# Orange-OpenSource/AIVC

Hardware: AMD Instinct MI355X
Metric: encode+decode fps @1080p YUV420 (RA GOP32) (higher is better)
Workload: dtype f32; 1 GPU; 1920x1080 8-bit YUV420, coding structure 1_GOP_32: one 128-frame clip = 4 intra-period units of 33 frames (132 coded frames, the last 4 repeat the last frame) encoded + decoded per step; synthetic random-init stand-in for model ms_ssim-4 (widths {'n2': 64, 'n': 128, 'c_y': 64, 'c_short': 64, 'c_z': 32, 'n_h': 128}), last analysis conv calibrated so that 6 (MOFNet) / 12 (CodecNet) of the 64 y featu; parallelism=single GPU

## Files before the change

### aivc_amd/csrc/conv_wino.hip

```cpp
#include <stdlib.h>

#include "mfma_util.h"

namespace aivc {

struct WinoArgs {
  aivc_conv_params p;
  int TH, TW;
  int nby, nbx;
  int gy;
  int total;
  int poly;
  int cpp_shift;
};

constexpr int WINO_RAW_STAGE = 11 * 1024;
constexpr int WINO_U_STAGE = 32 * 1024;
constexpr int WINO_V_QUAD = 1152;
constexpr int WINO_V_POS = 2 * WINO_V_QUAD;
constexpr int WINO_V_STAGE = 16 * WINO_V_POS;
constexpr int WINO_LDS = 2 * (WINO_RAW_STAGE + WINO_U_STAGE + WINO_V_STAGE);

__device__ __attribute__((aligned(4096))) float wino_zeros[1024];

template <int MODE>
__host__ __device__ constexpr bool wino_zero_pos(int pc, int i, int j) {
  if constexpr (MODE == 1) return ((pc >> 1) && i == 3) || ((pc & 1) && j == 3);
  if constexpr (MODE == 2) return ((pc >> 1) && i == 0) || ((pc & 1) && j == 0);
  return false;
}
template <int MODE>
__host__ __device__ constexpr uint32_t wino_pos_mask(int pc, int half) {
  uint32_t m = 0u;
  for (int q = 0; q < 8; ++q) m |= wino_zero_pos<MODE>(pc, 2 * half + (q >> 2), q & 3) ? 0u : 1u << q;
  return m;
}

struct WinoWalk {
  uint32_t x_lo, x_hi, slot, wg_per_xcd;
  __device__ __forceinline__ WinoWalk(uint32_t total, uint32_t nwg, uint32_t wg) {
    const uint32_t xcd = wg & 7u;
    slot = wg >> 3;
    const uint32_t per_xcd = (total + 7u) >> 3;
    wg_per_xcd = (nwg + 7u - xcd) >> 3;
    x_lo = xcd * per_xcd;
    x_hi = min(x_lo + per_xcd, total);
  }
  __device__ __forceinline__ uint32_t block_of(uint32_t k) const { return x_lo + slot + k * wg_per_xcd; }
  __device__ __forceinline__ uint32_t count() const { return x_lo + slot < x_hi ? (x_hi - x_lo - slot + wg_per_xcd - 1u) / wg_per_xcd : 0u; }
};

template <int MODE>
__global__ __launch_bounds__(512) void conv_wino_kernel(WinoArgs a) {
  constexpr bool POLY = MODE == 1, TC = MODE == 2;
  extern __shared__ __attribute__((aligned(16))) char wsmem[];
  char *raw = wsmem, *Us = wsmem + 2 * WINO_RAW_STAGE, *Vs = Us + 2 * WINO_U_STAGE;
  const uint32_t lds0 = (uint32_t)(uintptr_t)(__attribute__((address_space(3))) char *)wsmem;

  const aivc_conv_params &p = a.p;
  const int tid = threadIdx.x, lane = tid & 63;
  const int wave = __builtin_amdgcn_readfirstlane(tid >> 6);
  const int ph = wave >> 2, wm = (wave >> 1) & 1, wn = wave & 1;
  const int H = TC ? p.h_in : p.h_out, W = TC ? p.w_in : p.w_out, Hi = p.h_in, Wi = p.w_in, Cin = p.c_in, Cout = p.c_out;
  const int gyc = TC ? 4 * a.gy : a.gy;
  const int cpp_shift = a.cpp_shift, cpp_mask = (1 << a.cpp_shift) - 1;

  const WinoWalk walk((uint32_t)a.total, gridDim.x, blockIdx.x);
  const uint32_t n_mine = walk.count();
  if (n_mine == 0u) return;
  struct Desc {
    const float *xbase, *ubase;
    uint32_t r_off[2];
    int img, byi, bxi, cb;
  };
  int s_quad[2], s_py[2], s_px[2];
#pragma unroll
  for (int k = 0; k < 2; ++k) {
    int sl = 64 * (wave + 8 * k) + lane;
    sl = sl < 648 ? sl : 647;
    const int q2 = sl >> 1, plane = q2 / 81, rem = q2 - plane * 81, hy = rem / 9, hx = rem - hy * 9;
    s_quad[k] = sl & 1;
    s_py[k] = 2 * hy + (plane >> 1);
    s_px[k] = 2 * hx + (plane & 1);
  }
  const int nch = POLY ? 4 * (Cin >> 3) : (Cin >> 3);
  auto make_desc = [&](uint32_t blk) {
    Desc d;
    d.cb = (int)(blk % (uint32_t)gyc);
    uint32_t rest = blk / (uint32_t)gyc;
    d.bxi = (int)(rest % (uint32_t)a.nbx);
    rest /= (uint32_t)a.nbx;
    d.byi = (int)(rest % (uint32_t)a.nby);
    d.img = (int)(rest / (uint32_t)a.nby);
    d.xbase = p.x + (size_t)d.img * (size_t)Hi * Wi * Cin;
    d.ubase = p.w_wino + (size_t)d.cb * (size_t)nch * (WINO_U_STAGE / 4);
    if constexpr (MODE == 0) {
#pragma unroll
      for (int k = 0; k < 2; ++k) {
        const int iy = max(min(16 * d.byi - 1 + s_py[k], Hi - 1), 0), ix = max(min(16 * d.bxi - 1 + s_px[k], Wi - 1), 0);
        d.r_off[k] = ((uint32_t)(iy * Wi + ix) * (uint32_t)Cin + (uint32_t)(4 * s_quad[k])) * 4u;
      }
    }
    return d;
  };
  uint32_t iss_off[2];
  auto patch_offsets = [&](const Desc &d_, int ph2) {
    const int st = POLY ? 2 : 1, py = ph2 >> 1, px = ph2 & 1;
#pragma unroll
    for (int k = 0; k < 2; ++k) {
      const int iy = max(min(st * (16 * d_.byi - 1 + s_py[k]) + py, Hi - 1), 0), ix = max(min(st * (16 * d_.bxi - 1 + s_px[k]) + px, Wi - 1), 0);
      iss_off[k] = ((uint32_t)(iy * Wi + ix) * (uint32_t)Cin + (uint32_t)(4 * s_quad[k])) * 4u;
    }
  };
  uint64_t iss_addr[2];
  auto tc_addresses = [&](const Desc &d_) {
#pragma unroll
    for (int k = 0; k < 2; ++k) {
      const int iy = 16 * d_.byi - 1 + s_py[k], ix = 16 * d_.bxi - 1 + s_px[k];
      const bool in = iy >= 0 && iy < Hi && ix >= 0 && ix < Wi;
      const uint64_t a_in = (uint64_t)(uintptr_t)d_.xbase + ((uint64_t)((uint32_t)(iy * Wi + ix)) * (uint32_t)Cin + (uint32_t)(4 * s_quad[k])) * 4u;
      const uint64_t a_z = (uint64_t)(uintptr_t)wino_zeros + (uint32_t)(16 * s_quad[k]);
      iss_addr[k] = in ? a_in : a_z;
    }
  };
  Desc cur = make_desc(walk.block_of(0)), nxt = n_mine > 1u ? make_desc(walk.block_of(1)) : cur;

  const uint32_t r_dst = __builtin_amdgcn_readfirstlane(lds0 + (uint32_t)wave * 1024u);
  const uint32_t u_dst = __builtin_amdgcn_readfirstlane(lds0 + (uint32_t)(2 * WINO_RAW_STAGE) + (uint32_t)wave * 4096u);
  const uint32_t u_off = (uint32_t)(wave * 4096 + lane * 16);
  auto uniform_ptr = [](const float *q) -> const float * {
    const uint64_t v = (uint64_t)(uintptr_t)q;
    const uint32_t lo = __builtin_amdgcn_readfirstlane((uint32_t)v), hi = __builtin_amdgcn_readfirstlane((uint32_t)(v >> 32));
    return reinterpret_cast<const float *>((uintptr_t)(((uint64_t)hi << 32) | lo));
  };
  auto issue_raw = [&](const Desc &d_, int c) {
    const uint32_t d = r_dst + (uint32_t)((c & 1) * WINO_RAW_STAGE);
    if constexpr (TC) {
      if (c == 0) tc_addresses(d_);
      const uint32_t du = __builtin_amdgcn_readfirstlane(d);
      asm volatile("s_mov_b32 m0, %1\n\ts_nop 0\n\tglobal_load_lds_dwordx4 %0, off" : : "v"(iss_addr[0]), "s"(du) : "memory", "m0");
      if (wave < 3) asm volatile("s_mov_b32 m0, %1\n\ts_nop 0\n\tglobal_load_lds_dwordx4 %0, off" : : "v"(iss_addr[1]), "s"(du + 8192u) : "memory", "m0");
      iss_addr[0] += 32u;
      iss_addr[1] += 32u;
    } else {
      const float *src = d_.xbase + 8 * c;
      glds16(src, d_.r_off[0], d);
      if (wave < 3) glds16(src, d_.r_off[1], d + 8192u);
    }
  };
  auto issue_u = [&](const Desc &d_, int c) {
    const float *src = TC ? uniform_ptr(d_.ubase + (size_t)c * (WINO_U_STAGE / 4)) : d_.ubase + (size_t)c * (WINO_U_STAGE / 4);
    const uint32_t d = TC ? __builtin_amdgcn_readfirstlane(u_dst + (uint32_t)((c & 1) * WINO_U_STAGE)) : u_dst + (uint32_t)((c & 1) * WINO_U_STAGE);
    bool lo = true, hi = true;
    if constexpr (TC) {
      const int cls = d_.cb / a.gy, i = wave >> 1, j = 2 * (wave & 1);
      lo = !wino_zero_pos<MODE>(cls, i, j);
      hi = !wino_zero_pos<MODE>(cls, i, j + 1);
    }
    if (lo && hi) glds_piece<GLDS_BOTH>(src, u_off, d);
    else if (lo) glds_piece<GLDS_LO>(src, u_off, d);
    else if (hi) glds_piece<GLDS_HI>(src, u_off, d);
  };

  struct Prep {
    const float *r_src, *u_src;
    uint32_t flags;
  };
  auto prepare = [&](uint32_t kb, int cr, int cu) -> Prep {
    Prep q;
    const bool more = kb + 1u < n_mine;
    uint32_t fl = 0u;
    {
      const bool own = cr < nch;
      const int c = own ? cr : cr - nch;
      const Desc &d_ = own ? cur : nxt;
      if (own || more) {
        fl |= 1u;
        if ((c & cpp_mask) == 0) patch_offsets(d_, c >> cpp_shift);
      }
      q.r_src = uniform_ptr(d_.xbase + 8 * (c & cpp_mask));
    }
    {
      const bool own = cu < nch;
      const int c = own ? cu : cu - nch;
      const Desc &d_ = own ? cur : nxt;
      q.u_src = uniform_ptr(d_.ubase + (size_t)c * (WINO_U_STAGE / 4));
      if (own || more) {
        const int pc = c >> cpp_shift, i = wave >> 1, j = 2 * (wave & 1);
        if (!wino_zero_pos<MODE>(pc, i, j)) fl |= 2u;
        if (!wino_zero_pos<MODE>(pc, i, j + 1)) fl |= 4u;
      }
    }
    q.flags = __builtin_amdgcn_readfirstlane(fl);
    return q;
  };
  auto fire_raw = [&](auto STAGE, const Prep &q) {
    const uint32_t d = r_dst + (uint32_t)(decltype(STAGE)::value * WINO_RAW_STAGE);
    if (q.flags & 1u) {
      glds16(q.r_src, iss_off[0], d);
      if (wave < 3) glds16(q.r_src, iss_off[1], d + 8192u);
    }
  };
  auto fire_u = [&](auto STAGE, const Prep &q) {
    const uint32_t d = u_dst + (uint32_t)(decltype(STAGE)::value * WINO_U_STAGE);
    const uint32_t both = q.flags & 6u;
    if (both == 6u) glds_piece<GLDS_BOTH>(q.u_src, u_off, d);
    else if (both == 2u) glds_piece<GLDS_LO>(q.u_src, u_off, d);
    else if (both == 4u) glds_piece<GLDS_HI>(q.u_src, u_off, d);
  };

  const int l32 = lane & 31;
  const int t_grp = (l32 < 4 || (l32 >= 12 && l32 < 16) || (l32 >= 20 && l32 < 28)) ? 0 : 1;
  const int t_pos = t_grp == 0 ? (l32 < 4 ? l32 : (l32 < 16 ? l32 - 8 : l32 - 12)) : (l32 < 12 ? l32 - 4 : (l32 < 20 ? l32 - 8 : l32 - 16));
  const int t_quad = t_pos >> 3, t_tx = (t_pos & 7) ^ (t_grp << 2), t_ty = ((tid >> 6) & 1) * 4 + (lane >> 5) * 2 + t_grp;
  const int t_i = __builtin_amdgcn_readfirstlane(tid >> 7);
  const int t_ra = t_i == 0 ? 0 : (t_i == 2 ? 2 : 1), t_rb = t_i == 3 ? 3 : (t_i == 2 ? 1 : 2);
  const float t_si = t_i == 1 ? 1.0f : -1.0f;
  const int t_base = ((t_ty * 9 + t_tx) * 2 + t_quad) * 16;
  auto pix_off = [](int r, int c) { return (((r & 1) * 2 + (c & 1)) * 81 + (r >> 1) * 9 + (c >> 1)) * 32; };
  int t_oa[4], t_ob[4];
#pragma unroll
  for (int c = 0; c < 4; ++c) {
    t_oa[c] = t_base + pix_off(t_ra, c);
    t_ob[c] = t_base + pix_off(t_rb, c);
  }
  const int t_vdst = (4 * t_i) * WINO_V_POS + t_quad * WINO_V_QUAD + (t_ty * 8 + t_tx) * 16;
  float4 R[4];
  auto comb = [](const float4 &u, const float4 &v, float sgn) {
    float4 o;
    o.x = __builtin_fmaf(sgn, v.x, u.x);
    o.y = __builtin_fmaf(sgn, v.y, u.y);
    o.z = __builtin_fmaf(sgn, v.z, u.z);
    o.w = __builtin_fmaf(sgn, v.w, u.w);
    return o;
  };
  auto transform_step = [&](auto STAGE, auto STEP) {
    constexpr int st = decltype(STEP)::value, stage = decltype(STAGE)::value;
    const char *rs = raw + stage * WINO_RAW_STAGE;
    char *vd = Vs + stage * WINO_V_STAGE + t_vdst;
    if constexpr (st < 4) {
      const float4 xa = *reinterpret_cast<const float4 *>(rs + t_oa[st]), xb = *reinterpret_cast<const float4 *>(rs + t_ob[st]);
      R[st] = comb(xa, xb, t_si);
    } else if constexpr (st == 4) {
      *reinterpret_cast<float4 *>(vd) = comb(R[0], R[2], -1.0f);
    } else if constexpr (st == 5) {
      *reinterpret_cast<float4 *>(vd + WINO_V_POS) = comb(R[1], R[2], 1.0f);
    } else if constexpr (st == 6) {
      *reinterpret_cast<float4 *>(vd + 2 * WINO_V_POS) = comb(R[2], R[1], -1.0f);
    } else {
      *reinterpret_cast<float4 *>(vd + 3 * WINO_V_POS) = comb(R[1], R[3], -1.0f);
    }
  };
  auto transform0 = [&]() {
    using std::integral_constant;
    using Z = integral_constant<int, 0>;
    transform_step(Z{}, integral_constant<int, 0>{});
    transform_step(Z{}, integral_constant<int, 1>{});
    transform_step(Z{}, integral_constant<int, 2>{});
    transform_step(Z{}, integral_constant<int, 3>{});
    transform_step(Z{}, integral_constant<int, 4>{});
    transform_step(Z{}, integral_constant<int, 5>{});
    transform_step(Z{}, integral_constant<int, 6>{});
    transform_step(Z{}, integral_constant<int, 7>{});
  };

  floatx16 acc[8];
#pragma unroll
  for (int q = 0; q < 8; ++q)
#pragma unroll
    for (int r = 0; r < 16; ++r) acc[q][r] = 0.0f;
  const int hh = lane >> 5, l31 = lane & 31;
  const int a_rd = (8 * ph) * WINO_V_POS + hh * WINO_V_QUAD + (32 * wm + l31) * 16;
  const int b_rd = (8 * ph) * 2048 + hh * 1024 + (32 * wn + l31) * 16;
  auto multiply = [&](auto STAGE, auto FIRST, uint32_t pm, auto &&dma) {
    constexpr int stage = decltype(STAGE)::value;
    constexpr bool first = decltype(FIRST)::value;
    using NEXT = std::integral_constant<int, 1 - stage>;
    const char *va = Vs + stage * WINO_V_STAGE + a_rd, *ub = Us + stage * WINO_U_STAGE + b_rd;
    float4 af[2][2], bf[2][2];
    auto rd = [&](int set, int q) {
      af[set][0] = *reinterpret_cast<const float4 *>(va + q * WINO_V_POS);
      bf[set][0] = *reinterpret_cast<const float4 *>(ub + q * 2048);
      af[set][1] = *reinterpret_cast<const float4 *>(va + (q + 1) * WINO_V_POS);
      bf[set][1] = *reinterpret_cast<const float4 *>(ub + (q + 1) * 2048);
    };
    if constexpr (!TC) {
      if (ph) dma();
    }
    rd(0, 0);
    auto pair = [&](auto Q) {
      constexpr int q = decltype(Q)::value, set = (q >> 1) & 1;
      using std::integral_constant;
      if constexpr (q + 2 < 8) {
        if (MODE == 0 || (first && !TC) || (pm & (0xCu << q))) rd(1 - set, q + 2);
      }
      float4 ta[2], tb[2];
      auto reads = [&](auto S) {
        constexpr int st = decltype(S)::value;
        const char *rs = raw + (1 - stage) * WINO_RAW_STAGE;
        ta[0] = *reinterpret_cast<const float4 *>(rs + t_oa[st]);
        tb[0] = *reinterpret_cast<const float4 *>(rs + t_ob[st]);
        ta[1] = *reinterpret_cast<const float4 *>(rs + t_oa[st + 1]);
        tb[1] = *reinterpret_cast<const float4 *>(rs + t_ob[st + 1]);
      };
      auto finish = [&](auto S) {
        constexpr int st = decltype(S)::value;
        if constexpr (st < 4) {
          R[st] = comb(ta[0], tb[0], t_si);
          R[st + 1] = comb(ta[1], tb[1], t_si);
        } else {
          transform_step(NEXT{}, integral_constant<int, st>{});
          transform_step(NEXT{}, integral_constant<int, st + 1>{});
        }
      };
      if constexpr (q < 4) reads(Q);
      __builtin_amdgcn_sched_barrier(0);
      const float4 x0 = af[set][0], y0 = bf[set][0], x1 = af[set][1], y1 = bf[set][1];
      if constexpr (first && TC) {
        const floatx16 zero = {0.0f, 0.0f, 0.0f, 0.0f, 0.0f, 0.0f, 0.0f, 0.0f, 0.0f, 0.0f, 0.0f, 0.0f, 0.0f, 0.0f, 0.0f, 0.0f};
        if ((pm >> q) & 1u) acc[q] = mfma_oct1(x0, y0, zero);
        else acc[q] = __builtin_amdgcn_mfma_f32_32x32x2f32(0.0f, 0.0f, zero, 0, 0, 0);
        if ((pm >> (q + 1)) & 1u) acc[q + 1] = mfma_oct1(x1, y1, zero);
        else acc[q + 1] = __builtin_amdgcn_mfma_f32_32x32x2f32(0.0f, 0.0f, zero, 0, 0, 0);
      } else if constexpr (first) {
        const floatx16 zero = {0.0f, 0.0f, 0.0f, 0.0f, 0.0f, 0.0f, 0.0f, 0.0f, 0.0f, 0.0f, 0.0f, 0.0f, 0.0f, 0.0f, 0.0f, 0.0f};
        acc[q] = __builtin_amdgcn_mfma_f32_32x32x2f32(x0.x, y0.x, zero, 0, 0, 0);
        acc[q + 1] = __builtin_amdgcn_mfma_f32_32x32x2f32(x1.x, y1.x, zero, 0, 0, 0);
        acc[q] = __builtin_amdgcn_mfma_f32_32x32x2f32(x0.y, y0.y, acc[q], 0, 0, 0);
        acc[q + 1] = __builtin_amdgcn_mfma_f32_32x32x2f32(x1.y, y1.y, acc[q + 1], 0, 0, 0);
        acc[q] = __builtin_amdgcn_mfma_f32_32x32x2f32(x0.z, y0.z, acc[q], 0, 0, 0);
        acc[q + 1] = __builtin_amdgcn_mfma_f32_32x32x2f32(x1.z, y1.z, acc[q + 1], 0, 0, 0);
        acc[q] = __builtin_amdgcn_mfma_f32_32x32x2f32(x0.w, y0.w, acc[q], 0, 0, 0);
        acc[q + 1] = __builtin_amdgcn_mfma_f32_32x32x2f32(x1.w, y1.w, acc[q + 1], 0, 0, 0);
      } else {
        if (MODE == 0 || ((pm >> q) & 1u)) acc[q] = mfma_oct1(x0, y0, acc[q]);
        if (MODE == 0 || ((pm >> (q + 1)) & 1u)) acc[q + 1] = mfma_oct1(x1, y1, acc[q + 1]);
      }
      __builtin_amdgcn_sched_barrier(0);
      if constexpr (!TC && q == 0) {
        if (!ph) dma();
      }
      finish(Q);
      __builtin_amdgcn_sched_barrier(0);
    };
    using std::integral_constant;
    pair(integral_constant<int, 0>{});
    pair(integral_constant<int, 2>{});
    pair(integral_constant<int, 4>{});
    pair(integral_constant<int, 6>{});
  };

  auto issue_raw_at = [&](uint32_t kb, int c) {
    if (c < nch) issue_raw(cur, c);
    else if (kb + 1u < n_mine) issue_raw(nxt, c - nch);
  };
  auto issue_u_at = [&](uint32_t kb, int c) {
    if (c < nch) issue_u(cur, c);
    else if (kb + 1u < n_mine) issue_u(nxt, c - nch);
  };
  if constexpr (POLY) {
    const Prep q0 = prepare(0u, 0, 0);
    fire_raw(std::integral_constant<int, 0>{}, q0);
    fire_u(std::integral_constant<int, 0>{}, q0);
    fire_raw(std::integral_constant<int, 1>{}, prepare(0u, 1, 0));
  } else {
    issue_raw(cur, 0);
    issue_u(cur, 0);
    issue_raw_at(0u, 1);
  }
  asm volatile("s_waitcnt vmcnt(0)" ::: "memory");
  __builtin_amdgcn_s_barrier();
  transform0();
  asm volatile("s_waitcnt lgkmcnt(0)" ::: "memory");
  __builtin_amdgcn_s_barrier();
  const int act1 = p.act1, act2 = p.act2;
  for (uint32_t kb = 0; kb < n_mine; ++kb) {
    auto chunk = [&](auto STAGE, auto FIRST, int c) {
      Prep q;
      if constexpr (POLY) q = prepare(kb, c + 2, c + 1);
      auto dma = [&]() {
        if constexpr (POLY) {
          fire_raw(STAGE, q);
          fire_u(std::integral_constant<int, 1 - decltype(STAGE)::value>{}, q);
        } else {
          issue_raw_at(kb, c + 2);
          issue_u_at(kb, c + 1);
        }
      };
      uint32_t pm = 0xFFu;
      if constexpr (MODE != 0) {
        constexpr uint32_t ZCOL = 0xFFu ^ wino_pos_mask<MODE>(1, 0), ZROW = 0xFFu ^ wino_pos_mask<MODE>(2, POLY ? 1 : 0);
        static_assert(wino_pos_mask<MODE>(1, 1) == (0xFFu ^ ZCOL) && wino_pos_mask<MODE>(2, POLY ? 0 : 1) == 0xFFu &&
                      wino_pos_mask<MODE>(3, POLY ? 1 : 0) == (0xFFu ^ (ZCOL | ZROW)), "pm's two terms are the whole rule");
        const int pc = POLY ? c >> cpp_shift : cur.cb / a.gy;
        pm = 0xFFu & ~((pc & 1) ? ZCOL : 0u) & ~(((pc >> 1) && (POLY ? ph : !ph)) ? ZROW : 0u);
      }
      if constexpr (TC) dma();
      multiply(STAGE, FIRST, pm, dma);
      asm volatile("s_waitcnt vmcnt(0) lgkmcnt(0)" ::: "memory");
      __builtin_amdgcn_s_barrier();
    };
    {
      using std::integral_constant;
      using S0 = integral_constant<int, 0>;
      using S1 = integral_constant<int, 1>;
      chunk(S0{}, std::true_type{}, 0);
      chunk(S1{}, std::false_type{}, 1);
      for (int c = 2; c < nch; c += 2) {
        chunk(S0{}, std::false_type{}, c);
        chunk(S1{}, std::false_type{}, c + 1);
      }
    }

    floatx16 keep[2], give[2];
    auto fold = [&](auto PH) {
      constexpr int phc = decltype(PH)::value;
#pragma unroll
      for (int bb = 0; bb < 2; ++bb)
#pragma unroll
        for (int r = 0; r < 16; ++r) keep[bb][r] = give[bb][r] = 0.0f;
#pragma unroll
      for (int q = 0; q < 8; ++q) {
        const int i = 2 * phc + (q >> 2), j = q & 3;
        const int t0i = i < 3 ? 1 : 0, t1i = i == 0 ? 0 : (i == 1 ? 1 : -1);
        const int t0j = j < 3 ? 1 : 0, t1j = j == 0 ? 0 : (j == 1 ? 1 : -1);
#pragma unroll
        for (int o = 0; o < 4; ++o) {
          const int cf = ((o >> 1) ? t1i : t0i) * ((o & 1) ? t1j : t0j);
          floatx16 &dst = (o >> 1) == phc ? keep[o & 1] : give[o & 1];
          if (cf > 0) {
#pragma unroll
            for (int r = 0; r < 16; ++r) dst[r] = dst[r] + acc[q][r];
          } else if (cf < 0) {
#pragma unroll
            for (int r = 0; r < 16; ++r) dst[r] = dst[r] - acc[q][r];
          }
        }
      }
    };
    if (ph) fold(std::integral_constant<int, 1>{});
    else fold(std::integral_constant<int, 0>{});
    {
      float *xch = reinterpret_cast<float *>(Vs + WINO_V_STAGE) + wave * 1024;
      const float *theirs = reinterpret_cast<const float *>(Vs + WINO_V_STAGE) + (wave ^ 4) * 1024;
#pragma unroll
      for (int bb = 0; bb < 2; ++bb) {
#pragma unroll
        for (int r = 0; r < 16; ++r) xch[r * 64 + lane] = give[bb][r];
        asm volatile("s_waitcnt lgkmcnt(0)" ::: "memory");
        __builtin_amdgcn_s_barrier();
#pragma unroll
        for (int r = 0; r < 16; ++r) keep[bb][r] = keep[bb][r] + theirs[r * 64 + lane];
        asm volatile("s_waitcnt lgkmcnt(0)" ::: "memory");
        __builtin_amdgcn_s_barrier();
      }
    }

    {
      const float *__restrict__ g_mul = p.mul;
      const float *__restrict__ g_res = p.res;
      float *__restrict__ g_y = p.y;
      const int cls = TC ? cur.cb / a.gy : 0, pyc = cls >> 1, pxc = cls & 1;
      const int OS = TC ? 2 : 1;
      const int Wo_ = OS * W, Ho_ = OS * H;
      const int co = (TC ? cur.cb - cls * a.gy : cur.cb) * 64 + 32 * wn + l31;
      const bool has_bias = p.bias != nullptr;
      const float cbias = has_bias ? p.bias[co] : 0.0f;
      const int oy_w = 2 * (8 * cur.byi + 4 * wm) + ph;
      const bool inside_x = 16 * cur.bxi + 16 <= W;
      if (!g_mul && act1 != AIVC_ACT_SIGMOID) {
        const int cols_left = W - 16 * cur.bxi;
        typedef __attribute__((address_space(1))) char gchar;
        typedef __attribute__((address_space(1))) float gfloat;
        typedef __attribute__((address_space(1))) const float cgfloat;
        const uint32_t c4 = (uint32_t)Cout * 4u, sx = (uint32_t)OS * c4;
        uint32_t lane_b = (uint32_t)(2 * (8 * cur.bxi + 4 * hh)) * sx + (uint32_t)pxc * c4 + (uint32_t)co * 4u;
        asm volatile("" : "+v"(lane_b));
        const size_t img_b = (size_t)cur.img * (size_t)Ho_ * Wo_ * c4;
        auto rows = [&](auto RES, auto KIND, auto INSIDE) {
          constexpr bool has_res = decltype(RES)::value;
          constexpr bool edge = !decltype(INSIDE)::value;
          constexpr int kind = decltype(KIND)::value;
          bool ok[8];
#pragma unroll
          for (int rr = 0; rr < 4; ++rr)
#pragma unroll
            for (int b = 0; b < 2; ++b) ok[rr * 2 + b] = !edge || 2 * (4 * hh + rr) + b < cols_left;
#pragma unroll
          for (int rq = 0; rq < 4; ++rq) {
            const int oy = oy_w + 2 * rq;
            if (oy >= H) continue;
            const size_t row_b = img_b + (size_t)(OS * oy + pyc) * Wo_ * c4;
            gchar *yb = (gchar *)(uintptr_t)(reinterpret_cast<char *>(g_y) + row_b);
            const gchar *rb = (const gchar *)(uintptr_t)(reinterpret_cast<const char *>(g_res) + row_b);
            float rv[8];
            if constexpr (has_res) {
#pragma unroll
              for (int rr = 0; rr < 4; ++rr)
#pragma unroll
                for (int b = 0; b < 2; ++b)
                  rv[rr * 2 + b] = ok[rr * 2 + b] ? *reinterpret_cast<cgfloat *>(rb + lane_b + (uint32_t)((2 * rr + b) * 512) * (sx / 512u)) : 0.0f;
            }
#pragma unroll
            for (int rr = 0; rr < 4; ++rr)
#pragma unroll
              for (int b = 0; b < 2; ++b) {
                const int r = rq * 4 + rr;
                float v = keep[b][r];
                if (has_bias) v = v + cbias;
                if constexpr (kind == 1) v = __builtin_fmaxf(v, v * 0.01f);
                if constexpr (kind == 2) v = v > 0.0f ? v : 0.0f;
                if constexpr (has_res) v = v + rv[rr * 2 + b];
                if constexpr (kind == 3) v = v > 0.0f ? v : 0.0f;
                if constexpr (kind == 4) v = __builtin_fmaxf(v, v * 0.01f);
                if (ok[rr * 2 + b]) *reinterpret_cast<gfloat *>(yb + lane_b + (uint32_t)((2 * rr + b) * 512) * (sx / 512u)) = v;
              }
          }
        };
        using std::integral_constant;
        int kind = -1;
        if (act1 == AIVC_ACT_NONE && act2 == AIVC_ACT_NONE) kind = 0;
        else if (act2 == AIVC_ACT_NONE) kind = act1 == AIVC_ACT_LEAKY ? 1 : 2;
        else if (act1 == AIVC_ACT_NONE) kind = act2 == AIVC_ACT_RELU ? 3 : 4;
        if (kind >= 0 && sx % 512u == 0u) {
          auto go = [&](auto RES, auto INSIDE) {
            switch (kind) {
              case 0: rows(RES, integral_constant<int, 0>{}, INSIDE); break;
              case 1: rows(RES, integral_constant<int, 1>{}, INSIDE); break;
              case 2: rows(RES, integral_constant<int, 2>{}, INSIDE); break;
              case 3: rows(RES, integral_constant<int, 3>{}, INSIDE); break;
              default: rows(RES, integral_constant<int, 4>{}, INSIDE); break;
            }
          };
          if (inside_x) {
            if (g_res) go(integral_constant<bool, true>{}, integral_constant<bool, true>{});
            else go(integral_constant<bool, false>{}, integral_constant<bool, true>{});
          } else {
            if (g_res) go(integral_constant<bool, true>{}, integral_constant<bool, false>{});
            else go(integral_constant<bool, false>{}, integral_constant<bool, false>{});
          }
          goto epilogue_done;
        }
      }
      {
        const size_t ybase = (size_t)cur.img * (size_t)Ho_ * Wo_ * Cout + (size_t)co;
#pragma unroll
        for (int r = 0; r < 16; ++r) {
          const int t = (r & 3) + 8 * (r >> 2) + 4 * hh;
          const int oy = oy_w + 2 * (t >> 3), ox0 = 2 * (8 * cur.bxi + (t & 7));
          if (oy >= H) continue;
#pragma unroll
          for (int b = 0; b < 2; ++b) {
            const int ox = ox0 + b;
            if (ox >= W) continue;
            const size_t o = ybase + ((size_t)(OS * oy + pyc) * Wo_ + (size_t)(OS * ox + pxc)) * (size_t)Cout;
            float v = keep[b][r];
            if (has_bias) v = v + cbias;
            v = act_cheap(act1, v);
            if (g_mul) v = g_mul[o] * v;
            if (g_res) v = v + g_res[o];
            v = act_cheap(act2, v);
            g_y[o] = v;
          }
        }
      }
    epilogue_done:;
    }
    cur = nxt;
    if (kb + 2u < n_mine) nxt = make_desc(walk.block_of(kb + 2u));
  }
}

__device__ __forceinline__ void wino_g(double g0, double g1, double g2, double (&out)[4]) {
  out[0] = g0;
  out[1] = 0.5 * ((g0 + g1) + g2);
  out[2] = 0.5 * ((g0 - g1) + g2);
  out[3] = g2;
}

struct WinoForm3x3 {
  static constexpr int COUNT = 1;
  int co, ci, c_in;
  __device__ WinoForm3x3(size_t idx, int, int c_in_) : co((int)(idx / c_in_)), ci((int)(idx % c_in_)), c_in(c_in_) {}
  __device__ double tap(const float *w, int r, int l) const { return (double)w[(((size_t)co * 3 + r) * 3 + l) * c_in + ci]; }
  __device__ size_t out(int pos) const { return AIVC_WINO_U_INDEX(co, pos, ci, c_in); }
};
__device__ __forceinline__ double wino_tap5(const float *w, int co, int ci, int c_in, int ky, int kx) {
  return ky < 5 && kx < 5 ? (double)w[(((size_t)co * 5 + ky) * 5 + kx) * c_in + ci] : 0.0;
}
struct WinoFormPoly5 {
  static constexpr int COUNT = 4;
  int co, ci, c_in, phase;
  __device__ WinoFormPoly5(size_t idx, int, int c_in_)
      : co((int)(idx / ((size_t)4 * c_in_))), ci((int)((idx / 4) % c_in_)), c_in(c_in_), phase((int)(idx % 4)) {}
  __device__ double tap(const float *w, int r, int l) const { return wino_tap5(w, co, ci, c_in, 2 * r + (phase >> 1), 2 * l + (phase & 1)); }
  __device__ size_t out(int pos) const { return AIVC_WINO_U_INDEX(co, pos, phase * c_in + ci, 4 * c_in); }
};
struct WinoFormTconv5 {
  static constexpr int COUNT = 4;
  int co, ci, c_in, c_out, cls;
  __device__ WinoFormTconv5(size_t idx, int c_out_, int c_in_)
      : co((int)((idx / c_in_) % c_out_)), ci((int)(idx % c_in_)), c_in(c_in_), c_out(c_out_), cls((int)(idx / ((size_t)c_in_ * c_out_))) {}
  __device__ double tap(const float *w, int r, int l) const { return wino_tap5(w, co, ci, c_in, (cls >> 1) + 4 - 2 * r, (cls & 1) + 4 - 2 * l); }
  __device__ size_t out(int pos) const { return AIVC_WINO_U_INDEX(cls * c_out + co, pos, ci, c_in); }
};

template <class FORM>
__global__ void __launch_bounds__(256) winograd_weights_kernel(const float *w, int c_out, int c_in, float *u) {
  const size_t idx = (size_t)blockIdx.x * 256 + threadIdx.x;
  if (idx >= (size_t)c_out * c_in * FORM::COUNT) return;
  const FORM f(idx, c_out, c_in);
  double t[4][3], uu[4][4];
#pragma unroll
  for (int l = 0; l < 3; ++l) {
    double col[4];
    wino_g(f.tap(w, 0, l), f.tap(w, 1, l), f.tap(w, 2, l), col);
#pragma unroll
    for (int i = 0; i < 4; ++i) t[i][l] = col[i];
  }
#pragma unroll
  for (int i = 0; i < 4; ++i) wino_g(t[i][0], t[i][1], t[i][2], uu[i]);
#pragma unroll
  for (int i = 0; i < 4; ++i)
#pragma unroll
    for (int j = 0; j < 4; ++j) u[f.out(4 * i + j)] = (float)uu[i][j];
}

template <class FORM>
static int winograd_weights_launch(const char *what, const float *w, int c_out, int c_in, float *u, hipStream_t s) {
  hipLaunchKernelGGL(winograd_weights_kernel<FORM>, dim3(cdiv((size_t)c_out * c_in * FORM::COUNT, 256)), dim3(256), 0, s, w, c_out, c_in, u);
  return check_launch(what);
}
int winograd_weights(const float *w, int c_out, int c_in, float *u, hipStream_t s) {
  return winograd_weights_launch<WinoForm3x3>("winograd_weights", w, c_out, c_in, u, s);
}
int winograd_weights_poly5(const float *w, int c_out, int c_in, float *u, hipStream_t s) {
  return winograd_weights_launch<WinoFormPoly5>("winograd_weights_poly5", w, c_out, c_in, u, s);
}
int winograd_weights_tconv5(const float *w, int c_out, int c_in, float *u, hipStream_t s) {
  return winograd_weights_launch<WinoFormTconv5>("winograd_weights_tconv5", w, c_out, c_in, u, s);
}

struct WinoGrid {
  int gh, gw, nby, nbx;
  uint64_t blocks;
};
static WinoGrid wino_grid(const aivc_conv_params &p) {
  const bool tc = p.mode == AIVC_MODE_TCONV;
  const int gh = tc ? p.h_in : p.h_out, gw = tc ? p.w_in : p.w_out, nby = (gh + 15) / 16, nbx = (gw + 15) / 16;
  return {gh, gw, nby, nbx, (uint64_t)p.n * nby * nbx * ((uint64_t)p.c_out / 64) * (tc ? 4 : 1)};
}

bool conv2d_wino_supported(const aivc_conv_params &p) {
  if (!aivc_winograd_covers(&p) || p.gdn) return false;
  if ((uint64_t)p.h_in * p.w_in * p.c_in * 4u >= 0xFFFF0000ull) return false;
  if (p.mode == AIVC_MODE_TCONV && p.c_in > 960) return false;
  return wino_grid(p).blocks < 0x7FFFFFFFull;
}

int conv2d_wino_variant(const aivc_conv_params &p) { return p.mode == AIVC_MODE_TCONV ? 303 : (p.ksize == 5 ? 302 : 301); }

template <int MODE>
static int wino_launch(const WinoArgs &a, unsigned grid, hipStream_t s) {
  static LdsOptIn opt_in;
  if (!opt_in.raise(reinterpret_cast<const void *>(conv_wino_kernel<MODE>), WINO_LDS)) return check_launch("conv_wino lds attribute");
  hipLaunchKernelGGL(conv_wino_kernel<MODE>, dim3(grid), dim3(512), WINO_LDS, s, a);
  return check_launch("conv_wino");
}

int conv2d_wino(const aivc_conv_params &p, hipStream_t s) {
  if (!conv2d_wino_supported(p) || !p.w_wino) return AIVC_ERR_UNSUPPORTED;
  const bool tc = p.mode == AIVC_MODE_TCONV;
  WinoArgs a;
  a.p = p;
  a.poly = !tc && p.ksize == 5 ? 1 : 0;
  a.cpp_shift = 0;
  while ((8 << a.cpp_shift) < p.c_in) ++a.cpp_shift;
  const WinoGrid g = wino_grid(p);
  a.TH = (g.gh + 1) / 2;
  a.TW = (g.gw + 1) / 2;
  a.nby = g.nby;
  a.nbx = g.nbx;
  a.gy = p.c_out / 64;
  a.total = (int)g.blocks;
  static std::atomic<int> n_cu{0};
  if (n_cu.load(std::memory_order_relaxed) == 0) {
    int dev = 0, cus = 0;
    n_cu = hipGetDevice(&dev) == hipSuccess && hipDeviceGetAttribute(&cus, hipDeviceAttributeMultiprocessorCount, dev) == hipSuccess && cus > 0 ? cus : 256;
  }
  unsigned grid = (unsigned)n_cu.load(std::memory_order_relaxed);
  if ((unsigned)a.total < grid) grid = (unsigned)a.total;
  if (tc) return wino_launch<2>(a, grid, s);
  return a.poly ? wino_launch<1>(a, grid, s) : wino_launch<0>(a, grid, s);
}

}
```

Before: 100.3 frames/s.

## Tile 3x3 Winograd conv as pairs of 8-row strips instead of 16x16 blocks

For plain 3x3 convolutions the Winograd kernel now gives each workgroup two 8x16 output strips, which may come from different columns or images, instead of one 16x16 block. The raw input stage grows to hold two strips with their halos, and the epilogue takes its image and position per strip. The likely aim is finer tail granularity and better load balance on 1080p heights that are not multiples of 16, so fewer padded rows are computed. In exchange each strip pair carries more halo loads and uses more LDS. The epilogue setup is also hoisted and the goto removed, and a host helper is exported to list the strip pairs.

```diff
diff --git a/aivc_amd/csrc/conv_wino.hip b/aivc_amd/csrc/conv_wino.hip
--- a/aivc_amd/csrc/conv_wino.hip
+++ b/aivc_amd/csrc/conv_wino.hip
@@ -14,12 +14,21 @@
   int cpp_shift;
 };
 
-constexpr int WINO_RAW_STAGE = 11 * 1024;
+template <int MODE>
+constexpr int WINO_RAW_PLANE = MODE == 0 ? 45 : 81;
+template <int MODE>
+constexpr int WINO_RAW_SLOTS = MODE == 0 ? 720 : 648;
+template <int MODE>
+constexpr int WINO_RAW_STAGE = MODE == 0 ? 720 * 16 : 11 * 1024;
+constexpr int WINO_STRIP_SLOTS = 360;
 constexpr int WINO_U_STAGE = 32 * 1024;
 constexpr int WINO_V_QUAD = 1152;
 constexpr int WINO_V_POS = 2 * WINO_V_QUAD;
 constexpr int WINO_V_STAGE = 16 * WINO_V_POS;
-constexpr int WINO_LDS = 2 * (WINO_RAW_STAGE + WINO_U_STAGE + WINO_V_STAGE);
+template <int MODE>
+constexpr int WINO_LDS = 2 * (WINO_RAW_STAGE<MODE> + WINO_U_STAGE + WINO_V_STAGE);
+static_assert(WINO_LDS<0> <= 160 * 1024 && WINO_LDS<1> <= 160 * 1024 && WINO_LDS<2> <= 160 * 1024, "the stages of a workgroup fit the LDS of a CU");
+static_assert(WINO_RAW_STAGE<0> % 256 == 0 && WINO_RAW_STAGE<1> % 256 == 0, "the U and V stages keep their banks");
 
 __device__ __attribute__((aligned(4096))) float wino_zeros[1024];
 
@@ -50,11 +59,36 @@
   __device__ __forceinline__ uint32_t count() const { return x_lo + slot < x_hi ? (x_hi - x_lo - slot + wg_per_xcd - 1u) / wg_per_xcd : 0u; }
 };
 
+struct WinoPair {
+  int img[2], byi[2], bxi[2];
+};
+__host__ __device__ inline WinoPair wino_pair(uint32_t pair, int nby, int nbx, uint32_t n_strips) {
+  WinoPair q;
+  const uint32_t s0 = 2u * pair;
+  q.byi[0] = (int)(s0 % (uint32_t)nby);
+  const uint32_t col = s0 / (uint32_t)nby;
+  q.bxi[0] = (int)(col % (uint32_t)nbx);
+  q.img[0] = (int)(col / (uint32_t)nbx);
+  q.byi[1] = q.byi[0] + 1;
+  q.bxi[1] = q.bxi[0];
+  q.img[1] = q.img[0];
+  if (s0 + 1u >= n_strips) {
+    q.byi[1] = nby;
+  } else if (q.byi[1] == nby) {
+    q.byi[1] = 0;
+    if (++q.bxi[1] == nbx) {
+      q.bxi[1] = 0;
+      ++q.img[1];
+    }
+  }
+  return q;
+}
+
 template <int MODE>
 __global__ __launch_bounds__(512) void conv_wino_kernel(WinoArgs a) {
   constexpr bool POLY = MODE == 1, TC = MODE == 2;
   extern __shared__ __attribute__((aligned(16))) char wsmem[];
-  char *raw = wsmem, *Us = wsmem + 2 * WINO_RAW_STAGE, *Vs = Us + 2 * WINO_U_STAGE;
+  char *raw = wsmem, *Us = wsmem + 2 * WINO_RAW_STAGE<MODE>, *Vs = Us + 2 * WINO_U_STAGE;
   const uint32_t lds0 = (uint32_t)(uintptr_t)(__attribute__((address_space(3))) char *)wsmem;
 
   const aivc_conv_params &p = a.p;
@@ -69,35 +103,52 @@
   const uint32_t n_mine = walk.count();
   if (n_mine == 0u) return;
   struct Desc {
-    const float *xbase, *ubase;
+    const float *xbase[2], *ubase;
     uint32_t r_off[2];
-    int img, byi, bxi, cb;
-  };
-  int s_quad[2], s_py[2], s_px[2];
+    int img[2], byi[2], bxi[2], cb;
+  };
+  int s_quad[2], s_py[2], s_px[2], s_strip[2];
 #pragma unroll
   for (int k = 0; k < 2; ++k) {
     int sl = 64 * (wave + 8 * k) + lane;
-    sl = sl < 648 ? sl : 647;
-    const int q2 = sl >> 1, plane = q2 / 81, rem = q2 - plane * 81, hy = rem / 9, hx = rem - hy * 9;
+    sl = sl < WINO_RAW_SLOTS<MODE> ? sl : WINO_RAW_SLOTS<MODE> - 1;
+    s_strip[k] = MODE == 0 && sl >= WINO_STRIP_SLOTS ? 1 : 0;
+    if constexpr (MODE == 0) sl -= WINO_STRIP_SLOTS * s_strip[k];
+    const int q2 = sl >> 1, plane = q2 / WINO_RAW_PLANE<MODE>, rem = q2 - plane * WINO_RAW_PLANE<MODE>, hy = rem / 9, hx = rem - hy * 9;
     s_quad[k] = sl & 1;
     s_py[k] = 2 * hy + (plane >> 1);
     s_px[k] = 2 * hx + (plane & 1);
   }
+  const bool raw_second = MODE == 0 ? wave < 3 || (wave == 3 && lane < 16) : wave < 3;
+  const uint32_t n_strips = (uint32_t)p.n * (uint32_t)a.nby * (uint32_t)a.nbx;
   const int nch = POLY ? 4 * (Cin >> 3) : (Cin >> 3);
   auto make_desc = [&](uint32_t blk) {
     Desc d;
     d.cb = (int)(blk % (uint32_t)gyc);
     uint32_t rest = blk / (uint32_t)gyc;
-    d.bxi = (int)(rest % (uint32_t)a.nbx);
-    rest /= (uint32_t)a.nbx;
-    d.byi = (int)(rest % (uint32_t)a.nby);
-    d.img = (int)(rest / (uint32_t)a.nby);
-    d.xbase = p.x + (size_t)d.img * (size_t)Hi * Wi * Cin;
+    if constexpr (MODE == 0) {
+      const WinoPair pr = wino_pair(rest, a.nby, a.nbx, n_strips);
+#pragma unroll
+      for (int s = 0; s < 2; ++s) {
+        d.img[s] = pr.img[s];
+        d.byi[s] = pr.byi[s];
+        d.bxi[s] = pr.bxi[s];
+      }
+      d.xbase[0] = p.x + (size_t)d.img[0] * (size_t)Hi * Wi * Cin;
+      d.xbase[1] = p.x + (size_t)d.img[1] * (size_t)Hi * Wi * Cin;
+    } else {
+      d.bxi[0] = d.bxi[1] = (int)(rest % (uint32_t)a.nbx);
+      rest /= (uint32_t)a.nbx;
+      d.byi[0] = d.byi[1] = (int)(rest % (uint32_t)a.nby);
+      d.img[0] = d.img[1] = (int)(rest / (uint32_t)a.nby);
+      d.xbase[0] = d.xbase[1] = p.x + (size_t)d.img[0] * (size_t)Hi * Wi * Cin;
+    }
     d.ubase = p.w_wino + (size_t)d.cb * (size_t)nch * (WINO_U_STAGE / 4);
     if constexpr (MODE == 0) {
 #pragma unroll
       for (int k = 0; k < 2; ++k) {
-        const int iy = max(min(16 * d.byi - 1 + s_py[k], Hi - 1), 0), ix = max(min(16 * d.bxi - 1 + s_px[k], Wi - 1), 0);
+        const int sy = s_strip[k] ? d.byi[1] : d.byi[0], sx = s_strip[k] ? d.bxi[1] : d.bxi[0];
+        const int iy = max(min(8 * sy - 1 + s_py[k], Hi - 1), 0), ix = max(min(16 * sx - 1 + s_px[k], Wi - 1), 0);
         d.r_off[k] = ((uint32_t)(iy * Wi + ix) * (uint32_t)Cin + (uint32_t)(4 * s_quad[k])) * 4u;
       }
     }
@@ -108,7 +159,7 @@
     const int st = POLY ? 2 : 1, py = ph2 >> 1, px = ph2 & 1;
 #pragma unroll
     for (int k = 0; k < 2; ++k) {
-      const int iy = max(min(st * (16 * d_.byi - 1 + s_py[k]) + py, Hi - 1), 0), ix = max(min(st * (16 * d_.bxi - 1 + s_px[k]) + px, Wi - 1), 0);
+      const int iy = max(min(st * (16 * d_.byi[0] - 1 + s_py[k]) + py, Hi - 1), 0), ix = max(min(st * (16 * d_.bxi[0] - 1 + s_px[k]) + px, Wi - 1), 0);
       iss_off[k] = ((uint32_t)(iy * Wi + ix) * (uint32_t)Cin + (uint32_t)(4 * s_quad[k])) * 4u;
     }
   };
@@ -116,9 +167,9 @@
   auto tc_addresses = [&](const Desc &d_) {
 #pragma unroll
     for (int k = 0; k < 2; ++k) {
-      const int iy = 16 * d_.byi - 1 + s_py[k], ix = 16 * d_.bxi - 1 + s_px[k];
+      const int iy = 16 * d_.byi[0] - 1 + s_py[k], ix = 16 * d_.bxi[0] - 1 + s_px[k];
       const bool in = iy >= 0 && iy < Hi && ix >= 0 && ix < Wi;
-      const uint64_t a_in = (uint64_t)(uintptr_t)d_.xbase + ((uint64_t)((uint32_t)(iy * Wi + ix)) * (uint32_t)Cin + (uint32_t)(4 * s_quad[k])) * 4u;
+      const uint64_t a_in = (uint64_t)(uintptr_t)d_.xbase[0] + ((uint64_t)((uint32_t)(iy * Wi + ix)) * (uint32_t)Cin + (uint32_t)(4 * s_quad[k])) * 4u;
       const uint64_t a_z = (uint64_t)(uintptr_t)wino_zeros + (uint32_t)(16 * s_quad[k]);
       iss_addr[k] = in ? a_in : a_z;
     }
@@ -126,7 +177,7 @@
   Desc cur = make_desc(walk.block_of(0)), nxt = n_mine > 1u ? make_desc(walk.block_of(1)) : cur;
 
   const uint32_t r_dst = __builtin_amdgcn_readfirstlane(lds0 + (uint32_t)wave * 1024u);
-  const uint32_t u_dst = __builtin_amdgcn_readfirstlane(lds0 + (uint32_t)(2 * WINO_RAW_STAGE) + (uint32_t)wave * 4096u);
+  const uint32_t u_dst = __builtin_amdgcn_readfirstlane(lds0 + (uint32_t)(2 * WINO_RAW_STAGE<MODE>) + (uint32_t)wave * 4096u);
   const uint32_t u_off = (uint32_t)(wave * 4096 + lane * 16);
   auto uniform_ptr = [](const float *q) -> const float * {
     const uint64_t v = (uint64_t)(uintptr_t)q;
@@ -134,7 +185,7 @@
     return reinterpret_cast<const float *>((uintptr_t)(((uint64_t)hi << 32) | lo));
   };
   auto issue_raw = [&](const Desc &d_, int c) {
-    const uint32_t d = r_dst + (uint32_t)((c & 1) * WINO_RAW_STAGE);
+    const uint32_t d = r_dst + (uint32_t)((c & 1) * WINO_RAW_STAGE<MODE>);
     if constexpr (TC) {
       if (c == 0) tc_addresses(d_);
       const uint32_t du = __builtin_amdgcn_readfirstlane(d);
@@ -143,9 +194,14 @@
       iss_addr[0] += 32u;
       iss_addr[1] += 32u;
     } else {
-      const float *src = d_.xbase + 8 * c;
-      glds16(src, d_.r_off[0], d);
-      if (wave < 3) glds16(src, d_.r_off[1], d + 8192u);
+      const float *src0 = d_.xbase[0] + 8 * c, *src1 = d_.xbase[1] + 8 * c;
+      if (wave == 5) {
+        if (lane < WINO_STRIP_SLOTS - 5 * 64) glds16(src0, d_.r_off[0], d);
+        else glds16(src1, d_.r_off[0], d);
+      } else {
+        glds16(wave < 5 ? src0 : src1, d_.r_off[0], d);
+      }
+      if (raw_second) glds16(src1, d_.r_off[1], d + 8192u);
     }
   };
   auto issue_u = [&](const Desc &d_, int c) {
@@ -178,7 +234,7 @@
         fl |= 1u;
         if ((c & cpp_mask) == 0) patch_offsets(d_, c >> cpp_shift);
       }
-      q.r_src = uniform_ptr(d_.xbase + 8 * (c & cpp_mask));
+      q.r_src = uniform_ptr(d_.xbase[0] + 8 * (c & cpp_mask));
     }
     {
       const bool own = cu < nch;
@@ -195,7 +251,7 @@
     return q;
   };
   auto fire_raw = [&](auto STAGE, const Prep &q) {
-    const uint32_t d = r_dst + (uint32_t)(decltype(STAGE)::value * WINO_RAW_STAGE);
+    const uint32_t d = r_dst + (uint32_t)(decltype(STAGE)::value * WINO_RAW_STAGE<MODE>);
     if (q.flags & 1u) {
       glds16(q.r_src, iss_off[0], d);
       if (wave < 3) glds16(q.r_src, iss_off[1], d + 8192u);
@@ -216,8 +272,8 @@
   const int t_i = __builtin_amdgcn_readfirstlane(tid >> 7);
   const int t_ra = t_i == 0 ? 0 : (t_i == 2 ? 2 : 1), t_rb = t_i == 3 ? 3 : (t_i == 2 ? 1 : 2);
   const float t_si = t_i == 1 ? 1.0f : -1.0f;
-  const int t_base = ((t_ty * 9 + t_tx) * 2 + t_quad) * 16;
-  auto pix_off = [](int r, int c) { return (((r & 1) * 2 + (c & 1)) * 81 + (r >> 1) * 9 + (c >> 1)) * 32; };
+  const int t_base = MODE == 0 ? (t_ty >> 2) * (WINO_STRIP_SLOTS * 16) + (((t_ty & 3) * 9 + t_tx) * 2 + t_quad) * 16 : ((t_ty * 9 + t_tx) * 2 + t_quad) * 16;
+  auto pix_off = [](int r, int c) { return (((r & 1) * 2 + (c & 1)) * WINO_RAW_PLANE<MODE> + (r >> 1) * 9 + (c >> 1)) * 32; };
   int t_oa[4], t_ob[4];
 #pragma unroll
   for (int c = 0; c < 4; ++c) {
@@ -236,7 +292,7 @@
   };
   auto transform_step = [&](auto STAGE, auto STEP) {
     constexpr int st = decltype(STEP)::value, stage = decltype(STAGE)::value;
-    const char *rs = raw + stage * WINO_RAW_STAGE;
+    const char *rs = raw + stage * WINO_RAW_STAGE<MODE>;
     char *vd = Vs + stage * WINO_V_STAGE + t_vdst;
     if constexpr (st < 4) {
       const float4 xa = *reinterpret_cast<const float4 *>(rs + t_oa[st]), xb = *reinterpret_cast<const float4 *>(rs + t_ob[st]);
@@ -297,7 +353,7 @@
       float4 ta[2], tb[2];
       auto reads = [&](auto S) {
         constexpr int st = decltype(S)::value;
-        const char *rs = raw + (1 - stage) * WINO_RAW_STAGE;
+        const char *rs = raw + (1 - stage) * WINO_RAW_STAGE<MODE>;
         ta[0] = *reinterpret_cast<const float4 *>(rs + t_oa[st]);
         tb[0] = *reinterpret_cast<const float4 *>(rs + t_ob[st]);
         ta[1] = *reinterpret_cast<const float4 *>(rs + t_oa[st + 1]);
@@ -374,6 +430,11 @@
   asm volatile("s_waitcnt lgkmcnt(0)" ::: "memory");
   __builtin_amdgcn_s_barrier();
   const int act1 = p.act1, act2 = p.act2;
+  int kind = -1;
+  if (act1 == AIVC_ACT_SIGMOID) kind = -1;
+  else if (act1 == AIVC_ACT_NONE && act2 == AIVC_ACT_NONE) kind = 0;
+  else if (act2 == AIVC_ACT_NONE) kind = act1 == AIVC_ACT_LEAKY ? 1 : 2;
+  else if (act1 == AIVC_ACT_NONE) kind = act2 == AIVC_ACT_RELU ? 3 : 4;
   for (uint32_t kb = 0; kb < n_mine; ++kb) {
     auto chunk = [&](auto STAGE, auto FIRST, int c) {
       Prep q;
@@ -412,6 +473,40 @@
       }
     }
 
+    const float *__restrict__ g_mul = p.mul;
+    const float *__restrict__ g_res = p.res;
+    float *__restrict__ g_y = p.y;
+    const int cls = TC ? cur.cb / a.gy : 0, pyc = cls >> 1, pxc = cls & 1;
+    constexpr int OS = TC ? 2 : 1;
+    const int Wo_ = OS * W, Ho_ = OS * H;
+    const int co = (TC ? cur.cb - cls * a.gy : cur.cb) * 64 + 32 * wn + l31;
+    const bool has_bias = p.bias != nullptr;
+    const int e_img = MODE == 0 && wm ? cur.img[1] : cur.img[0], e_bxi = MODE == 0 && wm ? cur.bxi[1] : cur.bxi[0];
+    const int e_ty = MODE == 0 ? 4 * (wm ? cur.byi[1] : cur.byi[0]) : 8 * cur.byi[0] + 4 * wm;
+    const int oy_w = 2 * e_ty + ph;
+    const bool inside_x = 16 * e_bxi + 16 <= W;
+    const int cols_left = W - 16 * e_bxi;
+    typedef __attribute__((address_space(1))) char gchar;
+    typedef __attribute__((address_space(1))) float gfloat;
+    typedef __attribute__((address_space(1))) const float cgfloat;
+    const uint32_t c4 = (uint32_t)Cout * 4u, sx = (uint32_t)OS * c4;
+    uint32_t lane_b = (uint32_t)(2 * (8 * e_bxi + 4 * hh)) * sx + (uint32_t)pxc * c4 + (uint32_t)co * 4u;
+    asm volatile("" : "+v"(lane_b));
+    const size_t img_b = (size_t)e_img * (size_t)Ho_ * Wo_ * c4;
+    const bool fast = !g_mul && kind >= 0 && sx % 512u == 0u;
+    auto res_row = [&](auto INSIDE, int rq, float (&out)[8]) {
+      constexpr bool edge = !decltype(INSIDE)::value;
+      const size_t row_b = img_b + (size_t)(OS * (oy_w + 2 * rq) + pyc) * Wo_ * c4;
+      const gchar *rb = (const gchar *)(uintptr_t)(reinterpret_cast<const char *>(g_res) + row_b);
+#pragma unroll
+      for (int rr = 0; rr < 4; ++rr)
+#pragma unroll
+        for (int b = 0; b < 2; ++b) {
+          const bool ok = !edge || 2 * (4 * hh + rr) + b < cols_left;
+          out[rr * 2 + b] = ok ? *reinterpret_cast<cgfloat *>(rb + lane_b + (uint32_t)((2 * rr + b) * 512) * (sx / 512u)) : 0.0f;
+        }
+    };
+
     floatx16 keep[2], give[2];
     auto fold = [&](auto PH) {
       constexpr int phc = decltype(PH)::value;
@@ -457,30 +552,12 @@
     }
 
     {
-      const float *__restrict__ g_mul = p.mul;
-      const float *__restrict__ g_res = p.res;
-      float *__restrict__ g_y = p.y;
-      const int cls = TC ? cur.cb / a.gy : 0, pyc = cls >> 1, pxc = cls & 1;
-      const int OS = TC ? 2 : 1;
-      const int Wo_ = OS * W, Ho_ = OS * H;
-      const int co = (TC ? cur.cb - cls * a.gy : cur.cb) * 64 + 32 * wn + l31;
-      const bool has_bias = p.bias != nullptr;
       const float cbias = has_bias ? p.bias[co] : 0.0f;
-      const int oy_w = 2 * (8 * cur.byi + 4 * wm) + ph;
-      const bool inside_x = 16 * cur.bxi + 16 <= W;
-      if (!g_mul && act1 != AIVC_ACT_SIGMOID) {
-        const int cols_left = W - 16 * cur.bxi;
-        typedef __attribute__((address_space(1))) char gchar;
-        typedef __attribute__((address_space(1))) float gfloat;
-        typedef __attribute__((address_space(1))) const float cgfloat;
-        const uint32_t c4 = (uint32_t)Cout * 4u, sx = (uint32_t)OS * c4;
-        uint32_t lane_b = (uint32_t)(2 * (8 * cur.bxi + 4 * hh)) * sx + (uint32_t)pxc * c4 + (uint32_t)co * 4u;
-        asm volatile("" : "+v"(lane_b));
-        const size_t img_b = (size_t)cur.img * (size_t)Ho_ * Wo_ * c4;
+      if (fast) {
         auto rows = [&](auto RES, auto KIND, auto INSIDE) {
           constexpr bool has_res = decltype(RES)::value;
           constexpr bool edge = !decltype(INSIDE)::value;
-          constexpr int kind = decltype(KIND)::value;
+          constexpr int knd = decltype(KIND)::value;
           bool ok[8];
 #pragma unroll
           for (int rr = 0; rr < 4; ++rr)
@@ -492,15 +569,8 @@
             if (oy >= H) continue;
             const size_t row_b = img_b + (size_t)(OS * oy + pyc) * Wo_ * c4;
             gchar *yb = (gchar *)(uintptr_t)(reinterpret_cast<char *>(g_y) + row_b);
-            const gchar *rb = (const gchar *)(uintptr_t)(reinterpret_cast<const char *>(g_res) + row_b);
             float rv[8];
-            if constexpr (has_res) {
-#pragma unroll
-              for (int rr = 0; rr < 4; ++rr)
-#pragma unroll
-                for (int b = 0; b < 2; ++b)
-                  rv[rr * 2 + b] = ok[rr * 2 + b] ? *reinterpret_cast<cgfloat *>(rb + lane_b + (uint32_t)((2 * rr + b) * 512) * (sx / 512u)) : 0.0f;
-            }
+            if constexpr (has_res) res_row(INSIDE, rq, rv);
 #pragma unroll
             for (int rr = 0; rr < 4; ++rr)
 #pragma unroll
@@ -508,46 +578,38 @@
                 const int r = rq * 4 + rr;
                 float v = keep[b][r];
                 if (has_bias) v = v + cbias;
-                if constexpr (kind == 1) v = __builtin_fmaxf(v, v * 0.01f);
-                if constexpr (kind == 2) v = v > 0.0f ? v : 0.0f;
+                if constexpr (knd == 1) v = __builtin_fmaxf(v, v * 0.01f);
+                if constexpr (knd == 2) v = v > 0.0f ? v : 0.0f;
                 if constexpr (has_res) v = v + rv[rr * 2 + b];
-                if constexpr (kind == 3) v = v > 0.0f ? v : 0.0f;
-                if constexpr (kind == 4) v = __builtin_fmaxf(v, v * 0.01f);
+                if constexpr (knd == 3) v = v > 0.0f ? v : 0.0f;
+                if constexpr (knd == 4) v = __builtin_fmaxf(v, v * 0.01f);
                 if (ok[rr * 2 + b]) *reinterpret_cast<gfloat *>(yb + lane_b + (uint32_t)((2 * rr + b) * 512) * (sx / 512u)) = v;
               }
           }
         };
         using std::integral_constant;
-        int kind = -1;
-        if (act1 == AIVC_ACT_NONE && act2 == AIVC_ACT_NONE) kind = 0;
-        else if (act2 == AIVC_ACT_NONE) kind = act1 == AIVC_ACT_LEAKY ? 1 : 2;
-        else if (act1 == AIVC_ACT_NONE) kind = act2 == AIVC_ACT_RELU ? 3 : 4;
-        if (kind >= 0 && sx % 512u == 0u) {
-          auto go = [&](auto RES, auto INSIDE) {
-            switch (kind) {
-              case 0: rows(RES, integral_constant<int, 0>{}, INSIDE); break;
-              case 1: rows(RES, integral_constant<int, 1>{}, INSIDE); break;
-              case 2: rows(RES, integral_constant<int, 2>{}, INSIDE); break;
-              case 3: rows(RES, integral_constant<int, 3>{}, INSIDE); break;
-              default: rows(RES, integral_constant<int, 4>{}, INSIDE); break;
-            }
-          };
-          if (inside_x) {
-            if (g_res) go(integral_constant<bool, true>{}, integral_constant<bool, true>{});
-            else go(integral_constant<bool, false>{}, integral_constant<bool, true>{});
-          } else {
-            if (g_res) go(integral_constant<bool, true>{}, integral_constant<bool, false>{});
-            else go(integral_constant<bool, false>{}, integral_constant<bool, false>{});
+        auto go = [&](auto RES, auto INSIDE) {
+          switch (kind) {
+            case 0: rows(RES, integral_constant<int, 0>{}, INSIDE); break;
+            case 1: rows(RES, integral_constant<int, 1>{}, INSIDE); break;
+            case 2: rows(RES, integral_constant<int, 2>{}, INSIDE); break;
+            case 3: rows(RES, integral_constant<int, 3>{}, INSIDE); break;
+            default: rows(RES, integral_constant<int, 4>{}, INSIDE); break;
           }
-          goto epilogue_done;
+        };
+        if (inside_x) {
+          if (g_res) go(integral_constant<bool, true>{}, integral_constant<bool, true>{});
+          else go(integral_constant<bool, false>{}, integral_constant<bool, true>{});
+        } else {
+          if (g_res) go(integral_constant<bool, true>{}, integral_constant<bool, false>{});
+          else go(integral_constant<bool, false>{}, integral_constant<bool, false>{});
         }
-      }
-      {
-        const size_t ybase = (size_t)cur.img * (size_t)Ho_ * Wo_ * Cout + (size_t)co;
+      } else {
+        const size_t ybase = (size_t)e_img * (size_t)Ho_ * Wo_ * Cout + (size_t)co;
 #pragma unroll
         for (int r = 0; r < 16; ++r) {
           const int t = (r & 3) + 8 * (r >> 2) + 4 * hh;
-          const int oy = oy_w + 2 * (t >> 3), ox0 = 2 * (8 * cur.bxi + (t & 7));
+          const int oy = oy_w + 2 * (t >> 3), ox0 = 2 * (8 * e_bxi + (t & 7));
           if (oy >= H) continue;
 #pragma unroll
           for (int b = 0; b < 2; ++b) {
@@ -564,7 +626,6 @@
           }
         }
       }
-    epilogue_done:;
     }
     cur = nxt;
     if (kb + 2u < n_mine) nxt = make_desc(walk.block_of(kb + 2u));
@@ -647,7 +708,12 @@
 };
 static WinoGrid wino_grid(const aivc_conv_params &p) {
   const bool tc = p.mode == AIVC_MODE_TCONV;
-  const int gh = tc ? p.h_in : p.h_out, gw = tc ? p.w_in : p.w_out, nby = (gh + 15) / 16, nbx = (gw + 15) / 16;
+  const int gh = tc ? p.h_in : p.h_out, gw = tc ? p.w_in : p.w_out, nbx = (gw + 15) / 16;
+  if (!tc && p.ksize == 3) {
+    const int nsy = (gh + 7) / 8;
+    return {gh, gw, nsy, nbx, (((uint64_t)p.n * nsy * nbx + 1) / 2) * ((uint64_t)p.c_out / 64)};
+  }
+  const int nby = (gh + 15) / 16;
   return {gh, gw, nby, nbx, (uint64_t)p.n * nby * nbx * ((uint64_t)p.c_out / 64) * (tc ? 4 : 1)};
 }
 
@@ -658,13 +724,36 @@
   return wino_grid(p).blocks < 0x7FFFFFFFull;
 }
 
+}
+AIVC_EXPORT int aivc_wino_strip_list(int32_t n, int32_t h, int32_t w, int32_t *out) {
+  aivc_conv_params p = {};
+  p.mode = AIVC_MODE_CONV;
+  p.ksize = 3;
+  p.n = n;
+  p.h_out = h;
+  p.w_out = w;
+  p.c_out = 64;
+  const aivc::WinoGrid g = aivc::wino_grid(p);
+  if (out)
+    for (uint64_t k = 0; k < g.blocks; ++k) {
+      const aivc::WinoPair q = aivc::wino_pair((uint32_t)k, g.nby, g.nbx, (uint32_t)n * (uint32_t)g.nby * (uint32_t)g.nbx);
+      for (int s = 0; s < 2; ++s) {
+        out[6 * k + 3 * s] = q.img[s];
+        out[6 * k + 3 * s + 1] = q.byi[s];
+        out[6 * k + 3 * s + 2] = q.bxi[s];
+      }
+    }
+  return (int)g.blocks;
+}
+namespace aivc {
+
 int conv2d_wino_variant(const aivc_conv_params &p) { return p.mode == AIVC_MODE_TCONV ? 303 : (p.ksize == 5 ? 302 : 301); }
 
 template <int MODE>
 static int wino_launch(const WinoArgs &a, unsigned grid, hipStream_t s) {
   static LdsOptIn opt_in;
-  if (!opt_in.raise(reinterpret_cast<const void *>(conv_wino_kernel<MODE>), WINO_LDS)) return check_launch("conv_wino lds attribute");
-  hipLaunchKernelGGL(conv_wino_kernel<MODE>, dim3(grid), dim3(512), WINO_LDS, s, a);
+  if (!opt_in.raise(reinterpret_cast<const void *>(conv_wino_kernel<MODE>), WINO_LDS<MODE>)) return check_launch("conv_wino lds attribute");
+  hipLaunchKernelGGL(conv_wino_kernel<MODE>, dim3(grid), dim3(512), WINO_LDS<MODE>, s, a);
   return check_launch("conv_wino");
 }
 
```

Result: no change. 101.1 frames/s (median of 6 runs) (+0.8%).
